# kausaltech/reina-model

Measured on NVIDIA B200. Metric: agent-days/sec (HUS 1.7M), higher is better.
Workload: dtype int32/f32 state, f64 uniforms

## Files before the change

### reina_b200/csrc/contacts.cuh

```cuda
#ifndef REINA_B200_CONTACTS_CUH
#define REINA_B200_CONTACTS_CUH
#include "state.cuh"

#ifndef EX_THREADS
#define EX_THREADS 128
#endif
#ifndef EX_CTAS_PER_SM
#define EX_CTAS_PER_SM 24
#endif
#define EX_RESIDENT_PER_SM 12
#define EX_WARPS (EX_THREADS / 32)
#define EX_RCAP 256

__device__ __forceinline__ void expose_survivors(const Eng &G, int r, RepCtr *c, RepCtr *cd, const DevTable *tb, const uint2 *items, const uint32_t *sus,
                                                 Attempt *succ, uint32_t cap_succ, const uint32_t *ri, const uint32_t *rx, uint32_t head, uint32_t m, int lane) {
    const size_t base = (size_t)r * G.Npad;
    bool ok = false;
    uint32_t a = 0, t = 0, slot = 0;
    if ((uint32_t)lane < m) {
        const uint2 it = items[ri[(head + lane) & (EX_RCAP - 1)]];
        const uint32_t info = rx[(head + lane) & (EX_RCAP - 1)];
        const uint32_t row = (info >> 7) & 127u, kq = info >> 14;
        slot = info & 127u;
        a = it.x;
        const uint32_t age = (it.y >> 7) & 127u, dayidx = (it.y >> 14) & 31u, var = (it.y >> 20) & 3u;
        const rb_variant *v = &G.variants[var];
        float si = v->iot[dayidx];
        if ((it.y >> 19) & 1u) si = si * v->p_asymptomatic_infection;
        const u32x4 y = philox(c->seed, a, (uint32_t)c->day, PU_CONTACT2 | (slot << 8), 0);
        t = (uint32_t)tb->start[age][row] + y.x % (uint32_t)tb->size[age][row];
        if ((__ldg(&sus[t >> 5]) >> (t & 31)) & 1u) {
            const int tage = tb->susc_uniform[age][row] ? (int)tb->lo_age[age][row]
                                                        : age_in_band(G, (int32_t)t, tb->lo_age[age][row], tb->hi_age[age][row]);
            const float pr = (si * v->tab[RB_T_SUSCEPTIBILITY][tage]) * v->infectiousness_multiplier;
            if (((double)y.y * (1.0 / 4294967296.0)) * (double)kq < (double)pr * 256.0) {
                ok = true;
                const float mp = tb->mask_p[age][row];
                if (mp != 0.0f) {
                    const float ma = mp * v->p_mask_protects_others, mb = mp * v->p_mask_protects_wearer;
                    const float pm = (ma + mb) - ma * mb;
                    if (chance((double)y.z * (1.0 / 4294967296.0), pm)) ok = false;
                }
            }
        }
    }
    const uint32_t okm = __ballot_sync(0xffffffffu, ok);
    if (!okm) return;
    uint32_t b = 0;
    if (lane == 0) b = atomicAdd(&cd->n_succ, (uint32_t)__popc(okm));
    b = __shfl_sync(0xffffffffu, b, 0);
    if (!ok) return;
    const uint32_t idx = b + __popc(okm & ((1u << lane) - 1u));
    const unsigned long long key = ((unsigned long long)sweep_pos(G, r, c, a) << 7) | slot;
    if (idx < cap_succ) {
        succ[idx].cand = t; succ[idx].parent = a; succ[idx].key = key;
        if (!G.xbuf) atomicMin(&G.rec[base + t].winner, key);
    } else set_problem(cd, RB_OTHER_FAILURE);
}

__device__ __forceinline__ void expose_cta(const Eng &G, const int r, const uint32_t cta, const uint32_t ncta, int *s_place, uint32_t *ri, uint32_t *rx) {
    RepCtr *c = &G.ctr[r];
    const DevTable *tb = G.tables[c->epoch];
    const uint32_t n = min(c->n_items, G.cap_items);
    if (cta * blockDim.x >= n) return;
    if (threadIdx.x < RB_N_PLACES) s_place[threadIdx.x] = 0;
    __syncthreads();
    const uint2 *items = G.items + (size_t)r * G.cap_items;
    Attempt *succ = G.succ + (size_t)r * G.cap_succ;
    uint32_t cap_succ = G.cap_succ;
    RepCtr *cd = c;
    if (G.xbuf) { const XSlot x = xslot_of(G, G.rank, c->day); succ = x.succ; cap_succ = G.xcap_succ; cd = x.hdr; }
    const uint32_t *sus = G.sus + (size_t)r * G.sus_words;
    const uint32_t day = (uint32_t)c->day;
    const int lane = threadIdx.x & 31, warp = threadIdx.x >> 5;
    uint32_t head = 0, tail = 0;
    uint32_t places = 0;
    int since_flush = 0;
    const uint32_t stride = ncta * blockDim.x;
    uint2 nxt = make_uint2(0u, 0u);
    if (cta * blockDim.x + warp * 32 + lane < n) nxt = __ldcs(&items[cta * blockDim.x + warp * 32 + lane]);
    for (uint32_t i0 = cta * blockDim.x + warp * 32; i0 < n; i0 += stride) {
        const uint32_t i = i0 + lane;
        const bool valid = i < n;
        const uint2 it = nxt;
        if (i + stride < n) nxt = __ldcs(&items[i + stride]);
        uint32_t words[4] = {0, 0, 0, 0}, ncnt = 0, age = 0, grp = 0;
        int kq = 0;
        if (valid) {
            grp = it.y & 31u; ncnt = ((it.y >> 5) & 3u) + 1u; age = (it.y >> 7) & 127u;
            const rb_variant *v = &G.variants[(it.y >> 20) & 3u];
            float si = v->iot[(it.y >> 14) & 31u];
            if ((it.y >> 19) & 1u) si = si * v->p_asymptomatic_infection;
            const float p_upper = (si * v->reserved[0]) * v->infectiousness_multiplier;
            kq = (int)(p_upper * 256.0f) + 1;
            if (kq > 256) kq = 256;
            const u32x4 x = philox(c->seed, it.x, day, PU_CONTACT | (grp << 8), 0);
            words[0] = x.x; words[1] = x.y; words[2] = x.z; words[3] = x.w;
        }
        const int nrows = tb->n_rows[age];
        const uint32_t *cum24 = tb->cum24[age];
        const uint32_t *guide = tb->guide[age];
        uint32_t gd[4];
#pragma unroll
        for (uint32_t w = 0; w < 4; w++) gd[w] = w < ncnt ? __ldg(&guide[words[w] >> (32 - GUIDE_BITS)]) : 0u;
#pragma unroll
        for (uint32_t w = 0; w < 4; w++) {
            bool pass = false;
            uint32_t row = 0;
            if (w < ncnt) {
                const uint32_t word = words[w];
                const uint32_t k24 = word >> 8, g = gd[w], delta = (g >> 10) & 15u;
                row = g & 127u;
                uint32_t place = (g >> 7) & 7u;
                if (delta) {
                    if (delta < 15u) {
                        if ((k24 & ((1u << (24 - GUIDE_BITS)) - 1u)) >= (g >> 17)) { row += delta; place = (g >> 14) & 7u; }
                    } else {
                        while ((int)row < nrows - 1 && !(k24 < __ldg(&cum24[row]))) row++;
                        place = tb->place[age][row];
                    }
                }
                places += 1u << (5 * place);
                pass = (int)(word & 255u) < kq;
            }
            const unsigned m = __ballot_sync(0xffffffffu, pass);
            if (pass) {
                const uint32_t p = (tail + __popc(m & ((1u << lane) - 1u))) & (EX_RCAP - 1);
                ri[p] = i; rx[p] = (grp * 4u + w) | (row << 7) | ((uint32_t)kq << 14);
            }
            tail += __popc(m);
        }
        __syncwarp();
        while (tail - head >= 32) { expose_survivors(G, r, c, cd, tb, items, sus, succ, cap_succ, ri, rx, head, 32, lane); head += 32; }
        __syncwarp();
        if (++since_flush == 7) {
#pragma unroll
            for (int pl = 0; pl < RB_N_PLACES; pl++) { const uint32_t k = (places >> (5 * pl)) & 31u; if (k) atomicAdd(&s_place[pl], (int)k); }
            places = 0; since_flush = 0;
        }
    }
    if (tail != head) expose_survivors(G, r, c, cd, tb, items, sus, succ, cap_succ, ri, rx, head, tail - head, lane);
#pragma unroll
    for (int pl = 0; pl < RB_N_PLACES; pl++) { const uint32_t k = (places >> (5 * pl)) & 31u; if (k) atomicAdd(&s_place[pl], (int)k); }
    __syncthreads();
    if (threadIdx.x < RB_N_PLACES && s_place[threadIdx.x]) atomicAdd(&cd->daily_contacts[threadIdx.x], s_place[threadIdx.x]);
}
__global__ void __launch_bounds__(EX_THREADS, EX_RESIDENT_PER_SM) k_expose(Eng G) {
    __shared__ int s_place[RB_N_PLACES];
    __shared__ uint32_t s_ri[EX_WARPS][EX_RCAP], s_rx[EX_WARPS][EX_RCAP];
    const int warp = threadIdx.x >> 5;
    expose_cta(G, blockIdx.y + G.r0, blockIdx.x, gridDim.x, s_place, s_ri[warp], s_rx[warp]);
}

template <bool DRAIN>
__device__ __forceinline__ void resolve_part(const Eng &G, const int r, const uint32_t tid, const uint32_t nth) {
    RepCtr *c = &G.ctr[r];
    const size_t base = (size_t)r * G.Npad;
    const uint32_t n = min(c->n_succ, G.cap_succ);
    const Attempt *succ = G.succ + (size_t)r * G.cap_succ;
    const uint32_t stride = nth;
    const int list = (int)(c->lsel ^ 1u);
    const bool has_list = c->testing_mode == RB_ALL_WITH_SYMPTOMS_CT;
    for (uint32_t i = tid; i < n; i += 2 * stride) {
        const uint32_t j = i + stride;
        const bool two = j < n;
        const Attempt a0 = succ[i];
        Attempt a1 = a0;
        if (two) a1 = succ[j];
        const unsigned long long w0 = G.rec[base + a0.cand].winner;
        const uint32_t h0 = G.hot[base + a0.parent];
        unsigned long long w1 = KEY_IDLE; uint32_t h1 = 0;
        if (two) { w1 = G.rec[base + a1.cand].winner; h1 = G.hot[base + a1.parent]; }
#pragma unroll 1
        for (int k = 0; k < 2; k++) {
            const Attempt at = k ? a1 : a0;
            if ((k && !two) || (k ? w1 : w0) != at.key) continue;
            device_infect(G, r, c, (int32_t)at.cand, (int32_t)at.parent, k ? h1 : h0, 0, (int)(at.key & 127ull), false, list, has_list);
            G.rec[base + at.cand].winner = KEY_IDLE;
        }
    }
    if (tid == 0)
        c->wide_day = (c->n_events >= (uint32_t)G.wide_min || c->n_newq >= (uint32_t)G.wide_min) ? 1u : 0u;
    if (DRAIN) {
        const uint32_t nq = min(c->n_newq, G.cap_queue);
        const int32_t *qa = G.q_agent + ((size_t)r * 2 + (c->qsel ^ 1u)) * G.cap_queue;
        for (uint32_t i = tid; i < nq; i += nth) {
            const int32_t a = qa[i];
            const uint32_t h = G.hot[base + a];
            if (h & H_DET) set_problem(c, RB_WRONG_STATE);
            G.hot[base + a] = (h & ~H_QUEUED) | H_DET;
            mark_detected(G, r, a);
            atomicAdd(&c->drain_det[age_of(G, a)], 1);
        }
        if (tid == 0) c->drained = 1u;
    }
}
template <bool DRAIN>
__global__ void __launch_bounds__(256, 4) k_resolve(Eng G) {
    resolve_part<DRAIN>(G, blockIdx.y + G.r0, blockIdx.x * blockDim.x + threadIdx.x, gridDim.x * blockDim.x);
}

#endif
```

### reina_b200/csrc/run.cuh

```cuda
#ifndef REINA_B200_RUN_CUH
#define REINA_B200_RUN_CUH
#include "boundary.cuh"
#include "sweep.cuh"
#include "contacts.cuh"

#define RUN_THREADS 512
#define RUN_WARPS (RUN_THREADS / 32)
#ifndef RUN_CTAS_PER_SM
#define RUN_CTAS_PER_SM 2
#endif

union RunSmem {
    WarpRings rings[RUN_WARPS];
    struct { int place[8]; uint32_t ri[RUN_WARPS][EX_RCAP], rx[RUN_WARPS][EX_RCAP]; } ex;
    SmemSmall bd;
};

__device__ __forceinline__ void run_boundary(const Eng &G, const int r, RepCtr *c, RunSmem &S, Team &T, Team &B, const int kind) {
    const bool wide = B.ncta > 1 && (kind == 0 ? c->n_queue >= (uint32_t)G.wide_min : c->wide_day != 0u);
    Team L = team_of(c, 0, 1);
    Team &X = wide ? B : L;
    if (wide ? blockIdx.x < B.ncta : blockIdx.x == 0) {
        if (kind != 0) post_body(G, r, S.bd, X);
        if (kind == 2) team_sync(X);
        if (kind != 1) pre_body(G, r, S.bd, X);
    }
    team_sync(T);
}

__global__ void __launch_bounds__(RUN_THREADS, RUN_CTAS_PER_SM) k_run(Eng G, int n_days, int boundary_ctas) {
    __shared__ RunSmem S;
    const int r = blockIdx.y + G.r0;
    RepCtr *c = &G.ctr[r];
    const int lane = threadIdx.x & 31, warp = threadIdx.x >> 5;
    Team T = team_of(c, blockIdx.x, gridDim.x);
    T.bar = &c->run_bar;
    Team B = team_of(c, blockIdx.x, (uint32_t)boundary_ctas);
    const bool timing = G.dbg == 8 && blockIdx.x == 0 && threadIdx.x == 0;
    long long t0 = 0;
    auto lap = [&](int k) { if (timing) { long long t; asm volatile("mov.u64 %0, %%globaltimer;" : "=l"(t)); if (k >= 0) c->dbg_t[8 + k] += t - t0; t0 = t; } };
    lap(-1);
    for (int d = -1; d < n_days; d++) {
        const bool last = d == n_days - 1;
        if (d >= 0) {
            sweep_warp(G, r, blockIdx.x * RUN_WARPS + warp, gridDim.x * RUN_WARPS, S.rings[warp], lane);
            lap(1);
            team_sync(T);
            lap(2);
            expose_cta(G, r, blockIdx.x, gridDim.x, S.ex.place, S.ex.ri[warp], S.ex.rx[warp]);
            team_sync(T);
            lap(3);
            if (last) resolve_part<false>(G, r, blockIdx.x * RUN_THREADS + threadIdx.x, gridDim.x * RUN_THREADS);
            else resolve_part<true>(G, r, blockIdx.x * RUN_THREADS + threadIdx.x, gridDim.x * RUN_THREADS);
            team_sync(T);
            lap(4);
        }
        run_boundary(G, r, c, S, T, B, d < 0 ? 0 : (last ? 1 : 2));
        lap(d < 0 ? 0 : 5);
    }
    if (threadIdx.x == 0 && atomicAdd(&c->run_exit, 1u) == gridDim.x - 1u) { c->run_bar = 0u; c->wide_bar = 0u; c->run_exit = 0u; }
}

#endif
```

### reina_b200/csrc/sweep.cuh

```cuda
#ifndef REINA_B200_SWEEP_CUH
#define REINA_B200_SWEEP_CUH
#include "state.cuh"

#ifndef SW_THREADS
#define SW_THREADS 128
#endif
#define SW_WARPS (SW_THREADS / 32)
#define SW_RCAP 64
#ifndef SW_CTAS_PER_SM
#define SW_CTAS_PER_SM 9
#endif

struct WarpRings {
    uint32_t ea[SW_RCAP], ed[SW_RCAP];
    uint32_t ta[SW_RCAP], tw[SW_RCAP];
};

__device__ __forceinline__ uint32_t ring_push(uint32_t *ra, uint32_t *rb, uint32_t tail, bool want, uint32_t x, uint32_t y, int lane) {
    const uint32_t m = __ballot_sync(0xffffffffu, want);
    if (want) { uint32_t p = (tail + __popc(m & ((1u << lane) - 1u))) & (SW_RCAP - 1); ra[p] = x; rb[p] = y; }
    return tail + __popc(m);
}

__device__ __forceinline__ void seg_append(const Eng &G, RepCtr *c, uint2 *out, uint32_t &out_n, bool want, uint32_t a, uint32_t w, int lane) {
    const uint32_t m = __ballot_sync(0xffffffffu, want);
    if (want) {
        const uint32_t p = out_n + __popc(m & ((1u << lane) - 1u));
        if (p < G.seg_cap) out[p] = make_uint2(a, w); else set_problem(c, RB_OTHER_FAILURE);
    }
    out_n += __popc(m);
}

struct SweepOut {
    RepCtr *cd;
    unsigned long long *q_key; int32_t *q_agent; uint32_t cap_q;
    unsigned long long *ev_key; int32_t *ev_agent; uint32_t cap_ev;
    uint2 *upd; uint32_t cap_upd;
};
__device__ __forceinline__ SweepOut sweep_out(const Eng &G, int r, RepCtr *c) {
    SweepOut O;
    if (!G.xbuf) {
        const size_t qb = ((size_t)r * 2 + (c->qsel ^ 1u)) * G.cap_queue;
        O.cd = c; O.q_key = G.q_key + qb; O.q_agent = G.q_agent + qb; O.cap_q = G.cap_queue;
        O.ev_key = G.ev_key + (size_t)r * G.cap_events; O.ev_agent = G.ev_agent + (size_t)r * G.cap_events; O.cap_ev = G.cap_events;
        O.upd = nullptr; O.cap_upd = 0;
    } else {
        const XSlot x = xslot_of(G, G.rank, c->day);
        O.cd = x.hdr; O.q_key = x.q_key; O.q_agent = x.q_agent; O.cap_q = G.xcap_q;
        O.ev_key = x.ev_key; O.ev_agent = x.ev_agent; O.cap_ev = G.xcap_ev; O.upd = x.upd; O.cap_upd = G.xcap_upd;
    }
    return O;
}

__device__ __forceinline__ void stage_expose(const Eng &G, int r, RepCtr *c, RepCtr *cd, const DevTable *tb, const WarpRings &W, uint32_t head, uint32_t m,
                                             uint2 *items, int lane) {
    uint32_t ncont = 0, desc = 0, a = 0;
    if ((uint32_t)lane < m) {
        a = W.ea[(head + lane) & (SW_RCAP - 1)];
        desc = W.ed[(head + lane) & (SW_RCAP - 1)];
        bool detected = false;
        if (c->ct_ever) detected = (__ldg(&G.det[(size_t)r * G.sus_words + (a >> 5)]) >> (a & 31)) & 1u;
        if (!detected) {
            const int age = age_of(G, (int32_t)a);
            const int cls = (desc >> 22) & 1u;
            u32x4 x = philox(c->seed, a, (uint32_t)c->day, PU_NCONTACT, 0);
            const double u = u01d(x.x, x.y);
            const double *cdf = tb->ncdf[age][cls];
            const int limit = cls ? 5 : 100;
            const uint32_t ng = tb->nguide[age][cls][x.x >> 24];
            int k = (int)(ng & 127u);
            if (ng & 128u) while (k < limit && !(u < __ldg(&cdf[k]))) k++;
            ncont = (uint32_t)k;
            desc = (desc & ~(1u << 22)) | ((uint32_t)age << 7);
        }
    }
    const uint32_t cnt = (ncont + 3u) >> 2;
    uint32_t incl = cnt | (ncont << 16);
#pragma unroll
    for (int o = 1; o < 32; o <<= 1) { uint32_t t = __shfl_up_sync(0xffffffffu, incl, o); if (lane >= o) incl += t; }
    const uint32_t tot = __shfl_sync(0xffffffffu, incl, 31), wtot = tot & 0xffffu;
    if (wtot == 0) return;
    uint32_t gbase = 0;
    if (lane == 31) { gbase = atomicAdd(&c->n_items, wtot); atomicAdd(&cd->exposed_per_day, (int)(tot >> 16)); }
    gbase = __shfl_sync(0xffffffffu, gbase, 31);
    if (gbase + wtot > G.cap_items) { if (lane == 0) set_problem(cd, RB_OTHER_FAILURE); return; }
    uint2 *mine = items + gbase + ((incl & 0xffffu) - cnt);
    for (uint32_t g = 0; g < cnt; g++) {
        const uint32_t left = ncont - 4u * g;
        mine[g] = make_uint2(a, desc | g | (((left < 4u ? left : 4u) - 1u) << 5));
    }
}

__device__ __forceinline__ void emit_event(const Eng &G, int r, const SweepOut &O, RepCtr *c, int32_t a, int type) {
    uint32_t idx = atomicAdd(&O.cd->n_events, 1u);
    if (idx < O.cap_ev) {
        O.ev_key[idx] = ((unsigned long long)sweep_pos(G, r, c, (uint32_t)a) << 2) | (unsigned)type;
        O.ev_agent[idx] = a;
    } else set_problem(O.cd, RB_OTHER_FAILURE);
}

__device__ __forceinline__ uint32_t transition(const Eng &G, int r, RepCtr *c, const SweepOut &O, int32_t a, uint32_t h, uint32_t &lw) {
    RepCtr *cd = O.cd;
    const size_t base = (size_t)r * G.Npad;
    const int day = c->day;
    const int age = age_of(G, a);
    const uint32_t st = H_STATE(h), sev = H_SEV(h);
    const rb_variant *v = &G.variants[H_VAR(h)];
    uint32_t extra = 0;
    if (st == RB_INCUBATION) {
        float T = (sev == RB_FATAL)
            ? gamma_f(c->seed, (uint32_t)a, (uint32_t)day, PU_ONSET, v->onset_death_kappa, v->onset_death_theta)
            : gamma_f(c->seed, (uint32_t)a, (uint32_t)day, PU_ONSET, v->onset_recovery_kappa, v->onset_recovery_theta);
        float f = T;
        if (sev != RB_ASYMPTOMATIC && sev != RB_MILD) f = f * v->ratio_before_hospitalisation;
        const uint32_t dl = (uint32_t)clamp255(round_to_int(f));
        float w = 0.0f, u = 0.0f;
        if (sev == RB_SEVERE) w = T * (1.0f - v->ratio_before_hospitalisation);
        else if (sev == RB_CRITICAL || sev == RB_FATAL) {
            w = T * v->ratio_in_ward;
            u = ((1.0f - v->ratio_in_ward) - v->ratio_before_hospitalisation) * T;
        }
        const uint32_t wd = (uint32_t)clamp255(round_to_int(w)), ud = (uint32_t)clamp255(round_to_int(u));
        if (wd | ud) atomicOr(&G.rec[base + a].cold, (wd << 16) | (ud << 24));
        h = H_SET_DL(H_SET_STATE(h, RB_ILLNESS), dl);
        if (sev != RB_ASYMPTOMATIC && !(h & H_DET)) {
            bool q = false;
            const int mode = c->testing_mode;
            if (mode == RB_ALL_WITH_SYMPTOMS || mode == RB_ALL_WITH_SYMPTOMS_CT) q = true;
            else if (mode == RB_ONLY_SEVERE_SYMPTOMS) {
                if (sev >= RB_SEVERE) q = true;
                else {
                    u32x4 x = philox(c->seed, (uint32_t)a, (uint32_t)day, PU_SEEK, 0);
                    q = chance(u01d(x.x, x.y), c->p_detected_anyway);
                }
            }
            if (q && !(h & H_QUEUED)) {
                h |= H_QUEUED;
                uint32_t idx = atomicAdd(&cd->n_newq, 1u);
                if (idx < O.cap_q) {
                    O.q_key[idx] = QKEY_SWEEP | sweep_pos(G, r, c, (uint32_t)a);
                    O.q_agent[idx] = a;
                } else set_problem(cd, RB_OTHER_FAILURE);
            }
        }
        if (h & H_QUEUED) extra = H_DET;
    } else if (st == RB_ILLNESS) {
        if (sev == RB_FATAL) {
            h = H_SET_STATE(h, RB_DEAD) & ~H_LIST;
            count_add(cd, RB_A_INFECTED, age, -1); count_add(cd, RB_A_DEAD, age, 1); count_add(cd, RB_A_NON_HOSPITAL_DEATHS, age, 1);
        } else if (sev >= RB_SEVERE) {
            if (!(h & H_DET)) { h |= H_DET; count_add(cd, RB_A_DETECTED, age, 1); count_add(cd, RB_A_ALL_DETECTED, age, 1); }
            emit_event(G, r, O, c, a, EV_HOSP_CLAIM);
            extra = H_PEND;
        } else {
            h = H_SET_STATE(h, RB_RECOVERED) & ~H_LIST;
            count_add(cd, RB_A_INFECTED, age, -1); count_add(cd, RB_A_RECOVERED, age, 1);
        }
    } else {
        int type;
        if (st == RB_HOSPITALIZED && (sev == RB_CRITICAL || sev == RB_FATAL)) { type = EV_TO_ICU; extra = H_PEND; }
        else {
            type = st == RB_IN_ICU ? EV_ICU_RELEASE : EV_WARD_RELEASE;
            count_add(cd, st == RB_IN_ICU ? RB_A_IN_ICU : RB_A_IN_WARD, age, -1);
            count_add(cd, RB_A_INFECTED, age, -1);
            if (sev == RB_FATAL) { h = H_SET_STATE(h, RB_DEAD) & ~H_LIST; count_add(cd, RB_A_DEAD, age, 1); count_add(cd, RB_A_NON_HOSPITAL_DEATHS, age, 1); }
            else { h = H_SET_STATE(h, RB_RECOVERED) & ~H_LIST; count_add(cd, RB_A_RECOVERED, age, 1); }
        }
        emit_event(G, r, O, c, a, type);
    }
    lw = h | extra;
    return h;
}

__device__ __forceinline__ void stage_slow(const Eng &G, int r, RepCtr *c, RepCtr *cd, const WarpRings &W, uint32_t head, uint32_t m,
                                           uint32_t next, int lane) {
    const SweepOut O = sweep_out(G, r, c);
    const size_t base = (size_t)r * G.Npad;
    const bool on = (uint32_t)lane < m;
    bool keep = false, changed = false, removed = false;
    int infected_others = 0;
    uint32_t a = 0, lw = 0, h = 0;
    if (on) {
        a = W.ta[(head + lane) & (SW_RCAP - 1)];
        const uint32_t w = W.tw[(head + lane) & (SW_RCAP - 1)];
        const uint32_t hot = G.hot[base + a];
        if (w & H_PEND) {
            h = hot & ~H_FRESH;
            if (H_STATE(h) < RB_RECOVERED) { uint32_t dl = H_DL(h); if (dl > 0) dl--; h = H_SET_DL(h, dl); }
        } else h = (hot & ~(H_DAYS_MASK | H_FRESH)) | (w & H_DAYS_MASK);
        const uint32_t st = H_STATE(h);
        if (st >= RB_RECOVERED) {
            removed = true;
            infected_others = (int)(G.rec[base + a].cold & 0xffffu);
            G.hot[base + a] = hot | H_INCL;
        } else if (H_DL(h) == 0) {
            h = transition(G, r, c, O, (int32_t)a, h, lw);
            G.hot[base + a] = h;
            keep = true; changed = true;
        } else { lw = h; keep = true; }
    }
    const uint32_t rm = __ballot_sync(0xffffffffu, removed);
    if (rm) {
#pragma unroll
        for (int o = 16; o > 0; o >>= 1) infected_others += __shfl_xor_sync(0xffffffffu, infected_others, o);
        if (lane == 0) { atomicAdd(&cd->total_infectors, __popc(rm)); if (infected_others) atomicAdd(&cd->total_infections, infected_others); }
    }
    if (keep) list_add(G, r, cd, next, a, lw);
    if (O.upd) {
        const uint32_t mk = __ballot_sync(0xffffffffu, changed);
        uint32_t b = 0;
        if (lane == 0 && mk) b = atomicAdd(&O.cd->n_upd, (uint32_t)__popc(mk));
        b = __shfl_sync(0xffffffffu, b, 0);
        if (changed) {
            const uint32_t idx = b + __popc(mk & ((1u << lane) - 1u));
            if (idx < O.cap_upd) O.upd[idx] = make_uint2(a, h); else set_problem(O.cd, RB_OTHER_FAILURE);
        }
    }
}

__device__ __forceinline__ void stage_entry(const Eng &G, uint32_t &w, bool &keep, bool &want_e, bool &want_t, uint32_t &desc) {
    const uint32_t st = H_STATE(w);
    if ((w & H_PEND) || st >= RB_RECOVERED) { want_t = true; return; }
    if (w & H_FRESH) { w &= ~H_FRESH; keep = true; return; }
    const uint32_t sev = H_SEV(w), var = H_VAR(w);
    uint32_t dl = H_DL(w);
    if (st == RB_INCUBATION || st == RB_ILLNESS) {
        const int dayidx = st == RB_INCUBATION ? -(int)dl : (int)H_DOI(w);
        if (!(w & H_DET) && dayidx >= -10 && dayidx <= 10 && G.variants[var].iot[dayidx + 10] != 0.0f) {
            want_e = true;
            const uint32_t cls = (st == RB_ILLNESS && sev != RB_ASYMPTOMATIC) ? 1u : 0u;
            desc = ((uint32_t)(dayidx + 10) << 14) | ((sev == RB_ASYMPTOMATIC ? 1u : 0u) << 19) | (var << 20) | (cls << 22);
        }
        if (st == RB_ILLNESS) { uint32_t doi = H_DOI(w); if (doi < 31) doi++; w = H_SET_DOI(w, doi); }
    }
    if (dl > 0) dl--;
    w = H_SET_DL(w, dl);
    if (dl == 0) want_t = true; else keep = true;
}

__device__ __forceinline__ void sweep_warp(const Eng &G, const int r, const uint32_t first, const uint32_t n_warps, WarpRings &W, const int lane) {
    RepCtr *c = &G.ctr[r];
    const DevTable *tb = G.tables[c->epoch];
    uint2 *items = G.items + (size_t)r * G.cap_items;
    RepCtr *cd = !G.xbuf ? c : xslot_of(G, G.rank, c->day).hdr;
    const uint32_t cur = c->lsel;
    uint32_t e_head = 0, e_tail = 0, t_head = 0, t_tail = 0;

    uint2 cnt_next = make_uint2(0u, 0u);
    if (first < G.n_seg) cnt_next = *seg_count(G, r, cur, first);
    for (uint32_t seg = first; ; seg += n_warps) {
        const bool tail = seg >= G.n_seg;
        const uint2 cnt = cnt_next;
        cnt_next = make_uint2(0u, 0u);
        if (seg + n_warps < G.n_seg) cnt_next = *seg_count(G, r, cur, seg + n_warps);
        const uint32_t nf = min(cnt.x, G.seg_cap), n = min(cnt.x + cnt.y, G.seg_cap);
        const uint2 *in = seg_ptr(G, r, cur, tail ? 0u : seg);
        uint2 *out = seg_ptr(G, r, cur ^ 1u, tail ? 0u : seg);
        uint32_t out_n = 0;
        const uint32_t gap = G.seg_cap - n;
        auto entry = [&](uint32_t i) { return __ldcs(&in[i < nf ? i : i + gap]); };
        uint2 ent = make_uint2(0u, 0u);
        if ((uint32_t)lane < n) ent = entry(lane);
        uint32_t i0 = 0;
        bool again;
        do {
            if (i0 < n) {
                const bool valid = i0 + lane < n;
                const uint2 cur_ent = ent;
                if (i0 + 32 + lane < n) ent = entry(i0 + 32 + lane);
                bool keep = false, want_e = false, want_t = false;
                uint32_t w = cur_ent.y, desc = 0;
                if (valid) stage_entry(G, w, keep, want_e, want_t, desc);
                seg_append(G, cd, out, out_n, keep, cur_ent.x, w, lane);
                e_tail = ring_push(W.ea, W.ed, e_tail, want_e, cur_ent.x, desc, lane);
                t_tail = ring_push(W.ta, W.tw, t_tail, want_t, cur_ent.x, w, lane);
                __syncwarp();
            }
            const uint32_t e_av = e_tail - e_head, t_av = t_tail - t_head;
            if (e_av >= 32 || (tail && e_av)) { const uint32_t m = min(32u, e_av); stage_expose(G, r, c, cd, tb, W, e_head, m, items, lane); e_head += m; }
            if (t_av >= 32 || (tail && t_av)) { const uint32_t m = min(32u, t_av); stage_slow(G, r, c, cd, W, t_head, m, cur ^ 1u, lane); t_head += m; }
            __syncwarp();
            i0 += 32;
            again = tail ? (e_tail != e_head || t_tail != t_head) : i0 < n;
        } while (again);
        if (tail) break;
        if (lane == 0) seg_count(G, r, cur ^ 1u, seg)->x = out_n;
    }
}
__global__ void __launch_bounds__(SW_THREADS, SW_CTAS_PER_SM) k_sweep(Eng G) {
    __shared__ WarpRings s_rings[SW_WARPS];
    const int warp = threadIdx.x >> 5;
    sweep_warp(G, blockIdx.y + G.r0, blockIdx.x * SW_WARPS + warp, gridDim.x * SW_WARPS, s_rings[warp], threadIdx.x & 31);
}

__global__ void k_flush_lists(Eng G) {
    const int r = blockIdx.y;
    const RepCtr *c = &G.ctr[r];
    const size_t base = (size_t)r * G.Npad;
    const uint32_t cur = c->lsel;
    const int lane = threadIdx.x & 31;
    const uint32_t n_warps = gridDim.x * (blockDim.x >> 5);
    for (uint32_t seg = blockIdx.x * (blockDim.x >> 5) + (threadIdx.x >> 5); seg < G.n_seg; seg += n_warps) {
        const uint2 cnt = *seg_count(G, r, cur, seg);
        const uint32_t nf = min(cnt.x, G.seg_cap), n = min(cnt.x + cnt.y, G.seg_cap);
        const uint2 *in = seg_ptr(G, r, cur, seg);
        for (uint32_t i = lane; i < n; i += 32) {
            const uint2 e = in[i < nf ? i : i + (G.seg_cap - n)];
            if ((e.y & H_PEND) || H_STATE(e.y) >= RB_RECOVERED) continue;
            const uint32_t h = G.hot[base + e.x];
            G.hot[base + e.x] = (h & ~(H_DAYS_MASK | H_FRESH)) | (e.y & (H_DAYS_MASK | H_FRESH));
        }
    }
}
__global__ void k_rebuild_lists(Eng G) {
    const int r = blockIdx.y;
    RepCtr *c = &G.ctr[r];
    const size_t base = (size_t)r * G.Npad;
    const uint32_t cur = c->lsel;
    for (int a = blockIdx.x * blockDim.x + threadIdx.x; a < G.N; a += gridDim.x * blockDim.x) {
        if (!owns(G, (uint32_t)a)) continue;
        uint32_t h = G.hot[base + a];
        const uint32_t st = H_STATE(h);
        if (!((st >= RB_INCUBATION && st <= RB_IN_ICU) || (st >= RB_RECOVERED && !(h & H_INCL)))) continue;
        if (h & H_QUEUED) h |= H_DET;
        G.perm[base + a] = sweep_slot(G, c, (uint32_t)a);
        list_add(G, r, c, cur, (uint32_t)a, h);
    }
}
__global__ void k_clear_lists(Eng G) {
    const size_t n = (size_t)G.R * 2 * G.n_seg;
    for (size_t i = (size_t)blockIdx.x * blockDim.x + threadIdx.x; i < n; i += (size_t)gridDim.x * blockDim.x) G.seg_n[i] = make_uint2(0u, 0u);
}

#endif
```

Baseline: 740.0 billion.

## Move contact-count sampling from sweep into expose kernel, expand groups in-warp

The sweep stage now writes one item per infectious agent instead of expanding each agent into groups of four contacts. Contact-count sampling, the detection check and the exposed-per-day count move into the expose kernel, which expands contacts in-warp using a prefix scan and binary search, optionally through a dense compaction buffer. This shrinks the items array and its global traffic, and removes imbalance in the sweep stage. In exchange the expose kernel does more per-item work and shuffle-heavy expansion, and resident CTAs per SM drop from 12 to 10.

```diff
diff --git a/reina_b200/csrc/contacts.cuh b/reina_b200/csrc/contacts.cuh
--- a/reina_b200/csrc/contacts.cuh
+++ b/reina_b200/csrc/contacts.cuh
@@ -8,9 +8,25 @@
 #ifndef EX_CTAS_PER_SM
 #define EX_CTAS_PER_SM 24
 #endif
-#define EX_RESIDENT_PER_SM 12
+#ifndef EX_RESIDENT_PER_SM
+#define EX_RESIDENT_PER_SM 10
+#endif
 #define EX_WARPS (EX_THREADS / 32)
+#ifndef EX_DENSE
+#define EX_DENSE 0
+#endif
+#if EX_DENSE
+#define EX_CCAP 160
+#define EX_RCAP 64
+#else
+#define EX_CCAP 1
 #define EX_RCAP 256
+#endif
+
+struct ExBufs {
+    uint32_t cw[EX_CCAP], ci[EX_CCAP], cx[EX_CCAP];
+    uint32_t ri[EX_RCAP], rx[EX_RCAP];
+};
 
 __device__ __forceinline__ void expose_survivors(const Eng &G, int r, RepCtr *c, RepCtr *cd, const DevTable *tb, const uint2 *items, const uint32_t *sus,
                                                  Attempt *succ, uint32_t cap_succ, const uint32_t *ri, const uint32_t *rx, uint32_t head, uint32_t m, int lane) {
@@ -20,10 +36,10 @@
     if ((uint32_t)lane < m) {
         const uint2 it = items[ri[(head + lane) & (EX_RCAP - 1)]];
         const uint32_t info = rx[(head + lane) & (EX_RCAP - 1)];
-        const uint32_t row = (info >> 7) & 127u, kq = info >> 14;
+        const uint32_t row = (info >> 7) & 127u, kq = (info >> 14) & 511u, age = info >> 23;
         slot = info & 127u;
         a = it.x;
-        const uint32_t age = (it.y >> 7) & 127u, dayidx = (it.y >> 14) & 31u, var = (it.y >> 20) & 3u;
+        const uint32_t dayidx = (it.y >> 14) & 31u, var = (it.y >> 20) & 3u;
         const rb_variant *v = &G.variants[var];
         float si = v->iot[dayidx];
         if ((it.y >> 19) & 1u) si = si * v->p_asymptomatic_infection;
@@ -58,7 +74,26 @@
     } else set_problem(cd, RB_OTHER_FAILURE);
 }
 
-__device__ __forceinline__ void expose_cta(const Eng &G, const int r, const uint32_t cta, const uint32_t ncta, int *s_place, uint32_t *ri, uint32_t *rx) {
+__device__ __forceinline__ bool pick_contact(const DevTable *tb, const uint32_t word, uint32_t &info, uint32_t &places) {
+    const uint32_t age = info >> 23;
+    const uint32_t k24 = word >> 8, gd = __ldg(&tb->guide[age][word >> (32 - GUIDE_BITS)]), delta = (gd >> 10) & 15u;
+    uint32_t row = gd & 127u, place = (gd >> 7) & 7u;
+    if (delta) {
+        if (delta < 15u) {
+            if ((k24 & ((1u << (24 - GUIDE_BITS)) - 1u)) >= (gd >> 17)) { row += delta; place = (gd >> 14) & 7u; }
+        } else {
+            const int nrows = tb->n_rows[age];
+            while ((int)row < nrows - 1 && !(k24 < __ldg(&tb->cum24[age][row]))) row++;
+            place = tb->place[age][row];
+        }
+    }
+    places += 1u << (5 * place);
+    const bool pass = (word & 255u) < ((info >> 14) & 511u);
+    info |= row << 7;
+    return pass;
+}
+
+__device__ __forceinline__ void expose_cta(const Eng &G, const int r, const uint32_t cta, const uint32_t ncta, int *s_place, ExBufs &B) {
     RepCtr *c = &G.ctr[r];
     const DevTable *tb = G.tables[c->epoch];
     const uint32_t n = min(c->n_items, G.cap_items);
@@ -71,85 +106,141 @@
     RepCtr *cd = c;
     if (G.xbuf) { const XSlot x = xslot_of(G, G.rank, c->day); succ = x.succ; cap_succ = G.xcap_succ; cd = x.hdr; }
     const uint32_t *sus = G.sus + (size_t)r * G.sus_words;
+    const uint32_t *det = c->ct_ever ? G.det + (size_t)r * G.sus_words : nullptr;
     const uint32_t day = (uint32_t)c->day;
     const int lane = threadIdx.x & 31, warp = threadIdx.x >> 5;
+    const uint32_t lanes_below = (1u << lane) - 1u;
+    uint32_t cn = 0;
     uint32_t head = 0, tail = 0;
     uint32_t places = 0;
     int since_flush = 0;
+    int exposed = 0;
+    auto flush_places = [&]() {
+#pragma unroll
+        for (int pl = 0; pl < RB_N_PLACES; pl++) { const uint32_t k = (places >> (5 * pl)) & 31u; if (k) atomicAdd(&s_place[pl], (int)k); }
+        places = 0; since_flush = 0;
+    };
     const uint32_t stride = ncta * blockDim.x;
+    uint32_t i0 = cta * blockDim.x + warp * 32;
     uint2 nxt = make_uint2(0u, 0u);
-    if (cta * blockDim.x + warp * 32 + lane < n) nxt = __ldcs(&items[cta * blockDim.x + warp * 32 + lane]);
-    for (uint32_t i0 = cta * blockDim.x + warp * 32; i0 < n; i0 += stride) {
+    if (i0 + lane < n) nxt = __ldcs(&items[i0 + lane]);
+    for (;; i0 += stride) {
+        const bool last = i0 >= n;
         const uint32_t i = i0 + lane;
-        const bool valid = i < n;
         const uint2 it = nxt;
         if (i + stride < n) nxt = __ldcs(&items[i + stride]);
-        uint32_t words[4] = {0, 0, 0, 0}, ncnt = 0, age = 0, grp = 0;
-        int kq = 0;
-        if (valid) {
-            grp = it.y & 31u; ncnt = ((it.y >> 5) & 3u) + 1u; age = (it.y >> 7) & 127u;
+        uint32_t ncont = 0, meta = 0;
+        if (i < n && !(det && ((__ldg(&det[it.x >> 5]) >> (it.x & 31)) & 1u))) {
+            const int age = age_of(G, (int32_t)it.x);
+            const uint32_t cls = (it.y >> 22) & 1u;
+            const u32x4 x = philox(c->seed, it.x, day, PU_NCONTACT, 0);
+            const double u = u01d(x.x, x.y);
+            const double *cdf = tb->ncdf[age][cls];
+            const int limit = cls ? 5 : 100;
+            const uint32_t ng = tb->nguide[age][cls][x.x >> 24];
+            int k = (int)(ng & 127u);
+            if (ng & 128u) while (k < limit && !(u < __ldg(&cdf[k]))) k++;
+            ncont = (uint32_t)k;
             const rb_variant *v = &G.variants[(it.y >> 20) & 3u];
             float si = v->iot[(it.y >> 14) & 31u];
             if ((it.y >> 19) & 1u) si = si * v->p_asymptomatic_infection;
             const float p_upper = (si * v->reserved[0]) * v->infectiousness_multiplier;
-            kq = (int)(p_upper * 256.0f) + 1;
+            int kq = (int)(p_upper * 256.0f) + 1;
             if (kq > 256) kq = 256;
-            const u32x4 x = philox(c->seed, it.x, day, PU_CONTACT | (grp << 8), 0);
-            words[0] = x.x; words[1] = x.y; words[2] = x.z; words[3] = x.w;
-        }
-        const int nrows = tb->n_rows[age];
-        const uint32_t *cum24 = tb->cum24[age];
-        const uint32_t *guide = tb->guide[age];
-        uint32_t gd[4];
-#pragma unroll
-        for (uint32_t w = 0; w < 4; w++) gd[w] = w < ncnt ? __ldg(&guide[words[w] >> (32 - GUIDE_BITS)]) : 0u;
-#pragma unroll
-        for (uint32_t w = 0; w < 4; w++) {
-            bool pass = false;
-            uint32_t row = 0;
-            if (w < ncnt) {
-                const uint32_t word = words[w];
-                const uint32_t k24 = word >> 8, g = gd[w], delta = (g >> 10) & 15u;
-                row = g & 127u;
-                uint32_t place = (g >> 7) & 7u;
-                if (delta) {
-                    if (delta < 15u) {
-                        if ((k24 & ((1u << (24 - GUIDE_BITS)) - 1u)) >= (g >> 17)) { row += delta; place = (g >> 14) & 7u; }
-                    } else {
-                        while ((int)row < nrows - 1 && !(k24 < __ldg(&cum24[row]))) row++;
-                        place = tb->place[age][row];
+            meta = ncont | ((uint32_t)kq << 14) | ((uint32_t)age << 23);
+        }
+        uint32_t incl = ((ncont + 3u) >> 2) | (ncont << 16);
+#pragma unroll
+        for (int o = 1; o < 32; o <<= 1) { const uint32_t t = __shfl_up_sync(0xffffffffu, incl, o); if (lane >= o) incl += t; }
+        const uint32_t tot = __shfl_sync(0xffffffffu, incl, 31), ngrp = tot & 0xffffu;
+        exposed += (int)(tot >> 16);
+        incl &= 0xffffu;
+        for (uint32_t g0 = 0; ; g0 += 32) {
+            if (g0 < ngrp) {
+                const uint32_t g = g0 + lane;
+                uint32_t own = 0, before = 0;
+#pragma unroll
+                for (uint32_t s = 16; s; s >>= 1) { const uint32_t v = __shfl_sync(0xffffffffu, incl, own + s - 1); if (v <= g) { own += s; before = v; } }
+                const uint32_t om = __shfl_sync(0xffffffffu, meta, own), oa = __shfl_sync(0xffffffffu, it.x, own);
+                uint32_t words[4] = {0, 0, 0, 0}, nw = 0, info = 0;
+                if (g < ngrp) {
+                    const uint32_t grp = g - before, left = (om & 127u) - 4u * grp;
+                    nw = left < 4u ? left : 4u;
+                    info = (om & ~127u) | (grp * 4u);
+                    const u32x4 x = philox(c->seed, oa, day, PU_CONTACT | (grp << 8), 0);
+                    words[0] = x.x; words[1] = x.y; words[2] = x.z; words[3] = x.w;
+                }
+#if EX_DENSE
+#pragma unroll
+                for (uint32_t w = 0; w < 4; w++) {
+                    const uint32_t m = __ballot_sync(0xffffffffu, w < nw);
+                    if (w < nw) { const uint32_t p = cn + __popc(m & lanes_below); B.cw[p] = words[w]; B.ci[p] = i0 + own; B.cx[p] = info + w; }
+                    cn += __popc(m);
+                }
+#else
+#pragma unroll
+                for (uint32_t w = 0; w < 4; w++) {
+                    bool pass = false;
+                    uint32_t x = info + w;
+                    if (w < nw) pass = pick_contact(tb, words[w], x, places);
+                    const uint32_t m2 = __ballot_sync(0xffffffffu, pass);
+                    if (pass) { const uint32_t p = (tail + __popc(m2 & lanes_below)) & (EX_RCAP - 1); B.ri[p] = i0 + own; B.rx[p] = x; }
+                    tail += __popc(m2);
+                }
+                if (++since_flush == 7) flush_places();
+#endif
+                __syncwarp();
+            }
+            uint32_t pos = 0;
+            for (;;) {
+                const bool cround = cn - pos >= 32u || (last && cn != pos);
+                if (cround) {
+                    const uint32_t m = min(32u, cn - pos);
+                    bool pass = false;
+                    uint32_t rec = 0, info = 0;
+                    if ((uint32_t)lane < m) {
+                        const uint32_t word = B.cw[pos + lane];
+                        rec = B.ci[pos + lane]; info = B.cx[pos + lane];
+                        pass = pick_contact(tb, word, info, places);
                     }
-                }
-                places += 1u << (5 * place);
-                pass = (int)(word & 255u) < kq;
-            }
-            const unsigned m = __ballot_sync(0xffffffffu, pass);
-            if (pass) {
-                const uint32_t p = (tail + __popc(m & ((1u << lane) - 1u))) & (EX_RCAP - 1);
-                ri[p] = i; rx[p] = (grp * 4u + w) | (row << 7) | ((uint32_t)kq << 14);
-            }
-            tail += __popc(m);
-        }
-        __syncwarp();
-        while (tail - head >= 32) { expose_survivors(G, r, c, cd, tb, items, sus, succ, cap_succ, ri, rx, head, 32, lane); head += 32; }
-        __syncwarp();
-        if (++since_flush == 7) {
-#pragma unroll
-            for (int pl = 0; pl < RB_N_PLACES; pl++) { const uint32_t k = (places >> (5 * pl)) & 31u; if (k) atomicAdd(&s_place[pl], (int)k); }
-            places = 0; since_flush = 0;
-        }
-    }
-    if (tail != head) expose_survivors(G, r, c, cd, tb, items, sus, succ, cap_succ, ri, rx, head, tail - head, lane);
-#pragma unroll
-    for (int pl = 0; pl < RB_N_PLACES; pl++) { const uint32_t k = (places >> (5 * pl)) & 31u; if (k) atomicAdd(&s_place[pl], (int)k); }
+                    const uint32_t m2 = __ballot_sync(0xffffffffu, pass);
+                    if (pass) { const uint32_t p = (tail + __popc(m2 & lanes_below)) & (EX_RCAP - 1); B.ri[p] = rec; B.rx[p] = info; }
+                    tail += __popc(m2);
+                    pos += m;
+                    if (++since_flush == 31) flush_places();
+                    __syncwarp();
+                }
+                const bool sround = tail - head >= 32u || (last && !cround && tail != head);
+                if (sround) {
+                    const uint32_t m = min(32u, tail - head);
+                    expose_survivors(G, r, c, cd, tb, items, sus, succ, cap_succ, B.ri, B.rx, head, m, lane);
+                    head += m;
+                    __syncwarp();
+                }
+                if (!cround && !sround) break;
+            }
+            if (pos) {
+                const uint32_t left = cn - pos;
+                uint32_t w = 0, ii = 0, xx = 0;
+                if ((uint32_t)lane < left) { w = B.cw[pos + lane]; ii = B.ci[pos + lane]; xx = B.cx[pos + lane]; }
+                __syncwarp();
+                if ((uint32_t)lane < left) { B.cw[lane] = w; B.ci[lane] = ii; B.cx[lane] = xx; }
+                __syncwarp();
+                cn = left;
+            }
+            if (g0 + 32u >= ngrp) break;
+        }
+        if (last) break;
+    }
+    flush_places();
+    if (lane == 0 && exposed) atomicAdd(&cd->exposed_per_day, exposed);
     __syncthreads();
     if (threadIdx.x < RB_N_PLACES && s_place[threadIdx.x]) atomicAdd(&cd->daily_contacts[threadIdx.x], s_place[threadIdx.x]);
 }
 __global__ void __launch_bounds__(EX_THREADS, EX_RESIDENT_PER_SM) k_expose(Eng G) {
     __shared__ int s_place[RB_N_PLACES];
-    __shared__ uint32_t s_ri[EX_WARPS][EX_RCAP], s_rx[EX_WARPS][EX_RCAP];
-    const int warp = threadIdx.x >> 5;
-    expose_cta(G, blockIdx.y + G.r0, blockIdx.x, gridDim.x, s_place, s_ri[warp], s_rx[warp]);
+    __shared__ ExBufs s_bufs[EX_WARPS];
+    expose_cta(G, blockIdx.y + G.r0, blockIdx.x, gridDim.x, s_place, s_bufs[threadIdx.x >> 5]);
 }
 
 template <bool DRAIN>
diff --git a/reina_b200/csrc/run.cuh b/reina_b200/csrc/run.cuh
--- a/reina_b200/csrc/run.cuh
+++ b/reina_b200/csrc/run.cuh
@@ -12,7 +12,7 @@
 
 union RunSmem {
     WarpRings rings[RUN_WARPS];
-    struct { int place[8]; uint32_t ri[RUN_WARPS][EX_RCAP], rx[RUN_WARPS][EX_RCAP]; } ex;
+    struct { int place[8]; ExBufs bufs[RUN_WARPS]; } ex;
     SmemSmall bd;
 };
 
@@ -47,7 +47,7 @@
             lap(1);
             team_sync(T);
             lap(2);
-            expose_cta(G, r, blockIdx.x, gridDim.x, S.ex.place, S.ex.ri[warp], S.ex.rx[warp]);
+            expose_cta(G, r, blockIdx.x, gridDim.x, S.ex.place, S.ex.bufs[warp]);
             team_sync(T);
             lap(3);
             if (last) resolve_part<false>(G, r, blockIdx.x * RUN_THREADS + threadIdx.x, gridDim.x * RUN_THREADS);
diff --git a/reina_b200/csrc/sweep.cuh b/reina_b200/csrc/sweep.cuh
--- a/reina_b200/csrc/sweep.cuh
+++ b/reina_b200/csrc/sweep.cuh
@@ -52,43 +52,12 @@
     return O;
 }
 
-__device__ __forceinline__ void stage_expose(const Eng &G, int r, RepCtr *c, RepCtr *cd, const DevTable *tb, const WarpRings &W, uint32_t head, uint32_t m,
-                                             uint2 *items, int lane) {
-    uint32_t ncont = 0, desc = 0, a = 0;
-    if ((uint32_t)lane < m) {
-        a = W.ea[(head + lane) & (SW_RCAP - 1)];
-        desc = W.ed[(head + lane) & (SW_RCAP - 1)];
-        bool detected = false;
-        if (c->ct_ever) detected = (__ldg(&G.det[(size_t)r * G.sus_words + (a >> 5)]) >> (a & 31)) & 1u;
-        if (!detected) {
-            const int age = age_of(G, (int32_t)a);
-            const int cls = (desc >> 22) & 1u;
-            u32x4 x = philox(c->seed, a, (uint32_t)c->day, PU_NCONTACT, 0);
-            const double u = u01d(x.x, x.y);
-            const double *cdf = tb->ncdf[age][cls];
-            const int limit = cls ? 5 : 100;
-            const uint32_t ng = tb->nguide[age][cls][x.x >> 24];
-            int k = (int)(ng & 127u);
-            if (ng & 128u) while (k < limit && !(u < __ldg(&cdf[k]))) k++;
-            ncont = (uint32_t)k;
-            desc = (desc & ~(1u << 22)) | ((uint32_t)age << 7);
-        }
-    }
-    const uint32_t cnt = (ncont + 3u) >> 2;
-    uint32_t incl = cnt | (ncont << 16);
-#pragma unroll
-    for (int o = 1; o < 32; o <<= 1) { uint32_t t = __shfl_up_sync(0xffffffffu, incl, o); if (lane >= o) incl += t; }
-    const uint32_t tot = __shfl_sync(0xffffffffu, incl, 31), wtot = tot & 0xffffu;
-    if (wtot == 0) return;
+__device__ __forceinline__ void stage_expose(const Eng &G, RepCtr *c, RepCtr *cd, const WarpRings &W, uint32_t head, uint32_t m, uint2 *items, int lane) {
     uint32_t gbase = 0;
-    if (lane == 31) { gbase = atomicAdd(&c->n_items, wtot); atomicAdd(&cd->exposed_per_day, (int)(tot >> 16)); }
-    gbase = __shfl_sync(0xffffffffu, gbase, 31);
-    if (gbase + wtot > G.cap_items) { if (lane == 0) set_problem(cd, RB_OTHER_FAILURE); return; }
-    uint2 *mine = items + gbase + ((incl & 0xffffu) - cnt);
-    for (uint32_t g = 0; g < cnt; g++) {
-        const uint32_t left = ncont - 4u * g;
-        mine[g] = make_uint2(a, desc | g | (((left < 4u ? left : 4u) - 1u) << 5));
-    }
+    if (lane == 0) gbase = atomicAdd(&c->n_items, m);
+    gbase = __shfl_sync(0xffffffffu, gbase, 0);
+    if (gbase + m > G.cap_items) { if (lane == 0) set_problem(cd, RB_OTHER_FAILURE); return; }
+    if ((uint32_t)lane < m) items[gbase + lane] = make_uint2(W.ea[(head + lane) & (SW_RCAP - 1)], W.ed[(head + lane) & (SW_RCAP - 1)]);
 }
 
 __device__ __forceinline__ void emit_event(const Eng &G, int r, const SweepOut &O, RepCtr *c, int32_t a, int type) {
@@ -240,7 +209,6 @@
 
 __device__ __forceinline__ void sweep_warp(const Eng &G, const int r, const uint32_t first, const uint32_t n_warps, WarpRings &W, const int lane) {
     RepCtr *c = &G.ctr[r];
-    const DevTable *tb = G.tables[c->epoch];
     uint2 *items = G.items + (size_t)r * G.cap_items;
     RepCtr *cd = !G.xbuf ? c : xslot_of(G, G.rank, c->day).hdr;
     const uint32_t cur = c->lsel;
@@ -277,7 +245,7 @@
                 __syncwarp();
             }
             const uint32_t e_av = e_tail - e_head, t_av = t_tail - t_head;
-            if (e_av >= 32 || (tail && e_av)) { const uint32_t m = min(32u, e_av); stage_expose(G, r, c, cd, tb, W, e_head, m, items, lane); e_head += m; }
+            if (e_av >= 32 || (tail && e_av)) { const uint32_t m = min(32u, e_av); stage_expose(G, c, cd, W, e_head, m, items, lane); e_head += m; }
             if (t_av >= 32 || (tail && t_av)) { const uint32_t m = min(32u, t_av); stage_slow(G, r, c, cd, W, t_head, m, cur ^ 1u, lane); t_head += m; }
             __syncwarp();
             i0 += 32;
```

New measurement: 699.8 billion, median of 6. 5.4% lower.
